# at-wat/mcl_3dl

Hardware: AMD Instinct MI355X
Metric: particle·point evals/sec; filter-update Hz @ 4096 particles × 16k-pt scan (higher is better)
Workload: dtype f32

## Files before the change

### mcl_3dl_amd/capi.py

```python
import ctypes as C
import os

import numpy as np

_HERE = os.path.dirname(os.path.abspath(__file__))
LIB_PATH = os.environ.get("MCL3DL_HIP_LIB") or os.path.join(_HERE, "libmcl3dl_hip.so")

KERNEL_LIKELIHOOD, KERNEL_BEAM, KERNEL_PF, KERNEL_UPDATE, KERNEL_STAGE = 0, 1, 2, 3, 4
BEAM_STATUS = {0: "SHORT", 1: "HIT", 2: "LONG", 3: "TOTAL_REFLECTION"}

_f, _d, _sz, _u32, _u64, _i, _p = C.c_float, C.c_double, C.c_size_t, C.c_uint32, C.c_uint64, C.c_int, C.c_void_p

SIGNATURES = {
    "mcl3dl_hip_abi_version": (_i, []),
    "mcl3dl_hip_create": (_i, [C.POINTER(_p), _i]),
    "mcl3dl_hip_destroy": (None, [_p]),
    "mcl3dl_hip_last_error": (C.c_char_p, [_p]),
    "mcl3dl_hip_set_stream": (_i, [_p, _p]),
    "mcl3dl_hip_get_stream": (_p, [_p]),
    "mcl3dl_hip_synchronize": (_i, [_p]),
    "mcl3dl_hip_set_map": (_i, [_p, _p, _p, _sz, _u64, _p]),
    "mcl3dl_hip_set_likelihood_params": (_i, [_p, _f, _f, _f]),
    "mcl3dl_hip_set_beam_params": (_i, [_p, _f, _f, _f, _f, _f, _f, _f, _u32, _f, _u32, _i]),
    "mcl3dl_hip_set_beam_raycast": (_i, [_p, _i]),
# ... 929 lines not shown
    def pf_partial_device(self, d_weight, d_lik, d_beam, d_extra, d_ratio, n_p, d_packed, rank=0, world=1):
        self._check(self.lib.mcl3dl_hip_pf_partial_device(self.h, _ptr(d_weight), _ptr(d_lik), _ptr(d_beam),
                                                          _ptr(d_extra), _ptr(d_ratio), n_p, int(rank), int(world),
                                                          _ptr(d_packed)))

    def pf_apply_device(self, d_weight, n_p, d_packed, d_stats4, world=1):
        self._check(self.lib.mcl3dl_hip_pf_apply_device(self.h, _ptr(d_weight), n_p, int(world), _ptr(d_packed),
                                                        _ptr(d_stats4)))

    def set_kernel_timing(self, enable):
        self._check(self.lib.mcl3dl_hip_set_kernel_timing(self.h, int(bool(enable))))

    def reset_kernel_time(self):
        self._check(self.lib.mcl3dl_hip_reset_kernel_time(self.h))

    def kernel_time(self, kernel_id):
        ms, n = C.c_double(0), C.c_uint64(0)
        self._check(self.lib.mcl3dl_hip_get_kernel_time(self.h, kernel_id, C.byref(ms), C.byref(n)))
        return float(ms.value), int(n.value)

    def workload_stats(self, d_pose, n_p):
        st = np.zeros(6, np.float64)
        self._check(self.lib.mcl3dl_hip_workload_stats(self.h, _ptr(d_pose), n_p, _ptr(st)))
        return dict(sum_k=st[0], evals=st[1], dda_steps=st[2], dda_occupied=st[3], dda_tested=st[4], rays=st[5])

    def memory_footprint(self):
        b = np.zeros(8, np.uint64)
        self._check(self.lib.mcl3dl_hip_memory_footprint(self.h, _ptr(b)))
        return dict(lik_points=int(b[0]), lik_cells=int(b[1]), dda_bits=int(b[2]), dda_voxels=int(b[3]),
                    dda_points=int(b[4]), cand_table=int(b[5]), cand_start=int(b[6]), cand_points=int(b[7]))

    def set_option(self, name, value):
        self._check(self.lib.mcl3dl_hip_set_option(self.h, name.encode(), float(value)))

    def get_option(self, name):
        v = C.c_double(0)
        self._check(self.lib.mcl3dl_hip_get_option(self.h, name.encode(), C.byref(v)))
        return float(v.value)

    def index_stats(self):
        s = np.zeros(8, np.float64)
        self._check(self.lib.mcl3dl_hip_index_stats(self.h, _ptr(s)))
        return dict(bricks=int(s[0]), preliminary=int(s[1]), candidates=int(s[2]), build_ms=float(s[3]),
                    voxels_with_candidates=int(s[4]), voxels_with_overflow=int(s[5]), overflow_records=int(s[6]),
                    voxel_ratio=float(s[7]), voxels_over8=int(self.get_option("cand_voxels_over8")),
                    record_parts=int(self.get_option("cand_record_parts_in_use")),
                    packed_words=int(self.get_option("cand_packed_active")),
                    deferred_overflow=int(self.get_option("lik_defer_active")))
```

### mcl_3dl_amd/csrc/host_context.h

```cpp
#pragma once

namespace
{
struct DevBuf
{
  void* p = nullptr;
  size_t cap = 0;
  bool view = false;
  DevBuf() = default;
  DevBuf(const DevBuf&) = delete;
  DevBuf& operator=(const DevBuf&) = delete;
  ~DevBuf()
  {
    if (p && !view)
      (void)hipFree(p);
  }
  template <typename T>
  T* as() const
  {
    return static_cast<T*>(p);
  }
};

struct OrderedScan
// ... 89 lines not shown
  struct PinnedBlock
  {
    char* p;
    size_t bytes;
  };
  std::vector<PinnedBlock> pinned;
  bool is_pinned(const void* q, size_t bytes) const
  {
    const char* c = static_cast<const char*>(q);
    for (const PinnedBlock& b : pinned)
      if (c >= b.p && c + bytes <= b.p + b.bytes)
        return true;
    return false;
  }
  bool cand_aniso_active = false;
  double index_budget_bytes = 0.0;
  double cand_need_bytes = 0.0;
  double cand_edge_ratio[3] = { 0.5, 0.5, 0.5 };
  uint32_t cand_parts = 4;
  int n_cus = 256;
  double cand_over8 = 0;
  DevBuf cand_table, cand_start, cand_pts, cand_rec, cand_ovf;
  DevBuf cand_all_pts;
  CompileParams cand_cp{};
  long long cand_n_table = 0;
  uint32_t cand_n_bricks = 0, cand_n_ovf = 0, cand_ovf_leaked = 0;
  uint64_t cand_ovf_compactions = 0;
  size_t cand_n_points = 0;
  RecGrid rg{};
  double cand_stats[8] = { 0, 0, 0, 0, 0, 0, 0, 0 };
  DevBuf dda_bits, dda_start, dda_pts, dda_index;
  DevBuf dda_ov_key, dda_ov_pts, dda_ov_idx;
  bool dda_overlay_ok = false;
  uint64_t dda_overlay_updates = 0;
  DdaGeom dda_geom{};
  DevBuf map_dev;
  bool map_dev_valid = false;
  size_t map_dev_n = 0;
  double grid_build_ms[2] = { 0, 0 };
  double grid_build_wall_ms[2] = { 0, 0 };
  DdaGrid dg{};
  uint64_t footprint[8] = { 0, 0, 0, 0, 0, 0, 0, 0 };

  DevBuf scan_lik, scan_beam, origins, pow_table;
  DevBuf beam_origin;
  size_t n_s = 0, n_b = 0, n_o = 0;
// ... 553 lines not shown
```

### mcl_3dl_amd/csrc/host_map_compilers.h

```cpp
#pragma once

namespace
{
int build_lik_grid(mcl3dl_hip_ctx* ctx);
int build_dda_grid(mcl3dl_hip_ctx* ctx);
int ensure_map_dev(mcl3dl_hip_ctx* ctx);
int cloud_minmax(mcl3dl_hip_ctx* ctx, const float4* pts, long long n, float* host6, unsigned long long* host_cnt);

void kd_ray_radii(const mcl3dl_hip_ctx* ctx, float* grid_min, float* r1, float* r2)
{
  const float mn = std::min({ ctx->map_grid[0], ctx->map_grid[1], ctx->map_grid[2] });
  const float mx = std::max({ ctx->map_grid[0], ctx->map_grid[1], ctx->map_grid[2] });
  *grid_min = mn;
  *r1 = static_cast<float>(std::sqrt(2.0) * mx / 2.0);
  *r2 = static_cast<float>(mn * 2 + std::sqrt(2.0) * mx / 2.0);
}

bool lik_cell_is_beams(const mcl3dl_hip_ctx* ctx)
{
  return !ctx->lik_params_set && ctx->beam_raycast == 1;
}

float lik_cell_edge(const mcl3dl_hip_ctx* ctx)
{
// ... 506 lines not shown
  if (want_packed >= 0)
    out->packed = want_packed;
  else
    out->packed = (can_bound && ctx->opt.cand_packed && ctx->opt.cand_bound) ? 2 : (can_pack && ctx->opt.cand_packed) ? 1 : 0;
  TRY(scratch_alloc(ctx, out->d_ovf_data, 64ull * (n_ovf ? n_ovf : 1)));
  {
    const long long words = 16ll * (n_ovf ? n_ovf : 1);
    uint32_t sentinel_bits;
    const float sentinel = REC_SENTINEL;
    memcpy(&sentinel_bits, &sentinel, sizeof(sentinel_bits));
    hipLaunchKernelGGL(mc_fill_u32, dim3(static_cast<unsigned>((words + 255) / 256)), dim3(256), 0, ctx->stream,
                       static_cast<uint32_t*>(out->d_ovf_data.p), sentinel_bits, words);
  }
  hipLaunchKernelGGL(mc_write_records, dim3(blocks_v), dim3(256), 0, ctx->stream, pts,
                     static_cast<const uint32_t*>(d_pstart.p), static_cast<const uint32_t*>(d_prelim.p),
                     static_cast<const uint32_t*>(d_count.p), static_cast<const uint32_t*>(d_ovf.p), rec_out,
                     static_cast<float*>(out->d_ovf_data.p), n_vox, cap, out->packed, cp, bxyz,
                     static_cast<double>(ctx->match_dist_min));
  HIP_TRY(hipGetLastError());
  out->n_ovf = n_ovf;
  return 0;
}

constexpr int RC_OVER_BUDGET = 1;

int build_cand_grid_at(mcl3dl_hip_ctx* ctx, double voxel_ratio, uint32_t cap = 4)
{
  const unsigned long long rec_bytes = 16ull * cap;
  const size_t n = ctx->map_xyz.size() / 3;
  EventPairRaii evs;
  HIP_TRY(hipEventCreate(&evs.a));
  HIP_TRY(hipEventCreate(&evs.b));
  const hipEvent_t ev0 = evs.a, ev1 = evs.b;
  HIP_TRY(hipEventRecord(ev0, ctx->stream));
  TRY(ensure_map_dev(ctx));
  TRY(ensure(ctx, ctx->cand_all_pts, sizeof(float4) * n));
  hipLaunchKernelGGL(grid_rescale_kernel, dim3(static_cast<unsigned>((n + 255) / 256)), dim3(256), 0, ctx->stream,
                     ctx->map_dev.as<float4>(), static_cast<long long>(n), ctx->weight[0], ctx->weight[1], ctx->weight[2],
                     ctx->has_weight ? 1 : 0, ctx->cand_all_pts.as<float4>());
  float mm[6];
  unsigned long long n_finite = 0;
  TRY(cloud_minmax(ctx, ctx->cand_all_pts.as<float4>(), static_cast<long long>(n), mm, &n_finite));
  if (n_finite != n)
    return ctx->fail(-3, "%llu map point(s) are not finite", static_cast<unsigned long long>(n) - n_finite);
  const float* mn = mm;
  const float* mx = mm + 3;
// ... 17 lines not shown
  uint32_t n_bricks = 0;
  TRY(d2h(ctx, &n_bricks, static_cast<uint32_t*>(d_scan.p) + n_table, sizeof(uint32_t)));
  TRY(sync_stream(ctx));
  if (n_bricks == 0 || n_bricks > (1u << 22))
    return ctx->fail(-4, "candidate index: %u bricks", n_bricks);
  ctx->cand_need_bytes = static_cast<double>(rec_bytes) * 512.0 * n_bricks;
  if (ctx->opt.lik_index == 2 && ctx->index_budget_bytes > 0.0 && ctx->cand_need_bytes > ctx->index_budget_bytes)
    return RC_OVER_BUDGET;
  TRY(ensure(ctx, ctx->cand_table, sizeof(int) * (n_table + 1)));
  int* table = ctx->cand_table.as<int>();
  hipLaunchKernelGGL(mc_brick_ids, dim3(static_cast<unsigned>((n_table + 255) / 256)), dim3(256), 0, ctx->stream,
                     static_cast<const int*>(d_flag.p), static_cast<const uint32_t*>(d_scan.p), table, n_table);
  HIP_TRY(hipMemsetAsync(table + n_table, 0xff, sizeof(int), ctx->stream));
  TRY(scratch_alloc(ctx, d_bxyz, sizeof(int) * 3 * n_bricks));
  hipLaunchKernelGGL(mc_brick_coords, dim3(static_cast<unsigned>((n_table + 255) / 256)), dim3(256), 0, ctx->stream,
                     table, cp.nbx, cp.nby, n_table, static_cast<int*>(d_bxyz.p));
  const long long n_vox = static_cast<long long>(n_bricks) * 512;
  const bool records = ctx->opt.lik_index == 2;
  if (records)
    TRY(ensure(ctx, ctx->cand_rec, rec_bytes * static_cast<size_t>(n_vox)));
  CompileOutput co;
  TRY(compile_bricks(ctx, cp, pts, table, static_cast<const int*>(d_bxyz.p), n_bricks, records,
                     records ? ctx->cand_rec.as<float>() : nullptr, &co, cap));
  const unsigned long long total = co.total, kept = co.kept;
  ctx->cand_cp = cp;
  ctx->cand_n_table = n_table;
  ctx->cand_n_bricks = n_bricks;
  ctx->cand_n_points = n;
  if (records)
  {
    const uint32_t n_ovf = co.n_ovf;
    TRY(ensure(ctx, ctx->cand_ovf, 64ull * (n_ovf ? n_ovf : 1)));
    HIP_TRY(hipMemcpyAsync(ctx->cand_ovf.p, co.d_ovf_data.p, 64ull * (n_ovf ? n_ovf : 1), hipMemcpyDeviceToDevice,
                           ctx->stream));
    ctx->cand_n_ovf = n_ovf;
    ctx->cand_ovf_leaked = 0;
    HIP_TRY(hipEventRecord(ev1, ctx->stream));
    TRY(sync_stream(ctx));
    float ms2 = 0.f;
    HIP_TRY(hipEventSynchronize(ev1));
    HIP_TRY(hipEventElapsedTime(&ms2, ev0, ev1));
    RecGrid& g = ctx->rg;
    g.brick_table = table;
    g.rec = ctx->cand_rec.as<float4>();
    g.ovf = ctx->cand_ovf.as<float4>();
    g.ox = cp.ox;
// ... 239 lines not shown
                       c2, static_cast<const float4*>(dst), static_cast<int*>(d_dirty.p));
  }
  const unsigned blocks_tab = static_cast<unsigned>((n_table + 1 + 255) / 256);
  TRY(scratch_alloc(ctx, d_newflag, sizeof(uint32_t) * (n_table + 1)));
  TRY(scratch_alloc(ctx, d_dirtyrank, sizeof(uint32_t) * (n_table + 1)));
  hipLaunchKernelGGL(mc_new_brick_flags, dim3(blocks_tab), dim3(256), 0, ctx->stream, static_cast<const int*>(d_dirty.p),
                     ctx->cand_table.as<int>(), static_cast<uint32_t*>(d_newflag.p), n_table);
  HIP_TRY(hipMemsetAsync(d_dirtyrank.p, 0, sizeof(uint32_t) * (n_table + 1), ctx->stream));
  HIP_TRY(hipMemcpyAsync(d_dirtyrank.p, d_dirty.p, sizeof(int) * n_table, hipMemcpyDeviceToDevice, ctx->stream));
  TRY(device_exclusive_scan(ctx, static_cast<uint32_t*>(d_newflag.p), n_table + 1));
  TRY(device_exclusive_scan(ctx, static_cast<uint32_t*>(d_dirtyrank.p), n_table + 1));
  uint32_t n_new = 0, n_dirty = 0;
  TRY(d2h(ctx, &n_new, static_cast<uint32_t*>(d_newflag.p) + n_table, sizeof(uint32_t)));
  TRY(d2h(ctx, &n_dirty, static_cast<uint32_t*>(d_dirtyrank.p) + n_table, sizeof(uint32_t)));
  TRY(sync_stream(ctx));
  const uint32_t n_bricks_old = ctx->cand_n_bricks;
  if (n_dirty == 0)
  {
    if (stats5)
      stats5[5] = 6;
    ctx->cand_n_points = n_total;
    return 0;
  }
  if (static_cast<unsigned long long>(n_bricks_old) + n_new > (1u << 22))
  {
    if (stats5)
      stats5[5] = 5;
    ctx->cand_dirty = true;
    return 0;
  }
  if (ctx->cand_ovf_leaked > std::max<uint32_t>(4096u, ctx->cand_n_ovf / 2))
    TRY(compact_overflow(ctx));
  const uint32_t n_bricks = n_bricks_old + n_new;
  const uint32_t cap = ctx->cand_parts;
  const unsigned long long rec_bytes = 16ull * cap;
  TRY(ensure_keep(ctx, ctx->cand_rec, rec_bytes * 512 * n_bricks_old, rec_bytes * 512 * n_bricks));
  TRY(scratch_alloc(ctx, d_sub_table, sizeof(int) * n_table));
  TRY(scratch_alloc(ctx, d_sub_main, sizeof(int) * n_dirty));
  TRY(scratch_alloc(ctx, d_sub_bxyz, sizeof(int) * 3 * n_dirty));
  hipLaunchKernelGGL(mc_dirty_tables, dim3(blocks_tab), dim3(256), 0, ctx->stream, static_cast<const int*>(d_dirty.p),
                     static_cast<const uint32_t*>(d_newflag.p), static_cast<const uint32_t*>(d_dirtyrank.p), n_bricks_old,
                     cp.nbx, cp.nby, n_table, ctx->cand_table.as<int>(), static_cast<int*>(d_sub_table.p),
                     static_cast<int*>(d_sub_main.p), static_cast<int*>(d_sub_bxyz.p));
  cp.n_points = static_cast<int>(n_total);
  TRY(scratch_alloc(ctx, d_relflag, sizeof(uint32_t) * (n_total + 1)));
  hipLaunchKernelGGL(mc_relevant_points, dim3(static_cast<unsigned>((n_total + 1 + 255) / 256)), dim3(256), 0, ctx->stream,
                     cp, ctx->cand_all_pts.as<float4>(), static_cast<const int*>(d_dirty.p),
                     static_cast<uint32_t*>(d_relflag.p));
  TRY(device_exclusive_scan(ctx, static_cast<uint32_t*>(d_relflag.p), static_cast<long long>(n_total) + 1));
  uint32_t n_rel = 0;
  TRY(d2h(ctx, &n_rel, static_cast<uint32_t*>(d_relflag.p) + n_total, sizeof(uint32_t)));
  TRY(sync_stream(ctx));
  TRY(scratch_alloc(ctx, d_rel, sizeof(float4) * (n_rel ? n_rel : 1)));
  hipLaunchKernelGGL(mc_compact_points, dim3(static_cast<unsigned>((n_total + 255) / 256)), dim3(256), 0, ctx->stream,
                     ctx->cand_all_pts.as<float4>(), static_cast<const uint32_t*>(d_relflag.p), static_cast<int>(n_total),
                     static_cast<float4*>(d_rel.p));
  const long long n_sub_vox = static_cast<long long>(n_dirty) * 512;
  TRY(scratch_alloc(ctx, d_subrec, rec_bytes * static_cast<size_t>(n_sub_vox)));
  cp.n_points = static_cast<int>(n_rel);
  CompileOutput co;
  {
    const int rc = compile_bricks(ctx, cp, static_cast<const float4*>(d_rel.p), static_cast<const int*>(d_sub_table.p),
                                  static_cast<const int*>(d_sub_bxyz.p), n_dirty, true, static_cast<float*>(d_subrec.p), &co,
                                  cap, word_format(ctx->rg), ctx->cand_n_ovf);
    if (rc == 1)
    {
// ... 2 lines not shown
      ctx->cand_dirty = true;
      return 0;
    }
    if (rc != 0)
      return rc;
  }
  const uint32_t ovf_base = ctx->cand_n_ovf;
  if (co.n_ovf)
  {
    TRY(ensure_keep(ctx, ctx->cand_ovf, 64ull * ovf_base, 64ull * (static_cast<size_t>(ovf_base) + co.n_ovf)));
    HIP_TRY(hipMemcpyAsync(ctx->cand_ovf.as<char>() + 64ull * ovf_base, co.d_ovf_data.p, 64ull * co.n_ovf,
                           hipMemcpyDeviceToDevice, ctx->stream));
  }
  TempBuf d_orphan;
  TRY(scratch_alloc(ctx, d_orphan, sizeof(unsigned long long)));
  HIP_TRY(hipMemsetAsync(d_orphan.p, 0, sizeof(unsigned long long), ctx->stream));
  hipLaunchKernelGGL(mc_install_records, dim3(static_cast<unsigned>((n_sub_vox + 255) / 256)), dim3(256), 0, ctx->stream,
                     static_cast<const float4*>(d_subrec.p), static_cast<const int*>(d_sub_main.p), ovf_base, n_bricks_old,
                     n_sub_vox, ctx->cand_rec.as<float4>(), static_cast<unsigned long long*>(d_orphan.p), cap, ctx->rg.packed,
                     ctx->rg.count_shift, ctx->rg.count_is_records);
  HIP_TRY(hipGetLastError());
  unsigned long long orphaned = 0;
  TRY(d2h(ctx, &orphaned, d_orphan.p, sizeof(orphaned)));
  HIP_TRY(hipEventRecord(ev1, ctx->stream));
  TRY(sync_stream(ctx));
  float ms = 0.f;
  HIP_TRY(hipEventSynchronize(ev1));
  HIP_TRY(hipEventElapsedTime(&ms, ev0, ev1));
  ctx->cand_n_bricks = n_bricks;
  ctx->cand_n_ovf = ovf_base + co.n_ovf;
  ctx->cand_ovf_leaked += static_cast<uint32_t>(orphaned);
  ctx->cand_n_points = n_total;
  ctx->rg.brick_table = ctx->cand_table.as<int>();
  ctx->rg.rec = ctx->cand_rec.as<float4>();
  ctx->rg.ovf = ctx->cand_ovf.as<float4>();
  ctx->rg.off32_ok = (rec_bytes * 512 * n_bricks < (1ull << 32)) ? 1 : 0;
  ctx->rg.rec_bytes32 = bytes32(rec_bytes * 512 * n_bricks);
  ctx->rg.ovf_bytes32 = bytes32(64ull * (ctx->cand_n_ovf ? ctx->cand_n_ovf : 1));
  ctx->footprint[6] = rec_bytes * 512 * n_bricks;
  ctx->footprint[7] = 64ull * ctx->cand_n_ovf;
  ctx->cand_stats[0] = n_bricks;
  ctx->cand_stats[6] = ctx->cand_n_ovf;
  if (stats5)
  {
    stats5[0] = n_dirty;
    stats5[1] = n_new;
// ... 9 lines not shown
```

### mcl_3dl_amd/csrc/host_measure.h

```cpp
#pragma once
#include <type_traits>

namespace
{
int ensure_structures(mcl3dl_hip_ctx* ctx, bool need_lik, bool need_dda, bool need_cells = false)
{
  if (!ctx->has_map)
    return ctx->fail(-5, "no map: call mcl3dl_hip_set_map first");
  bool built = false;
  if (need_lik && ctx->opt.lik_index == 0 && !need_cells && !ctx->lik_params_set && (ctx->lik_cell_from_beam || lik_cell_is_beams(ctx)))
  {
    ctx->lik_params_set = true;
    if (ctx->lik_cell_from_beam)
      ctx->lik_dirty = ctx->lik_base_dirty = true;
  }
  if (need_lik && (ctx->opt.lik_index == 0 || need_cells) && ctx->lik_dirty)
  {
    TRY(build_lik_grid(ctx));
    built = true;
  }
  if (need_lik && ctx->opt.lik_index >= 1 && !need_cells && ctx->cand_dirty)
  {
    TRY(build_cand_grid(ctx));
    built = true;
// ... 961 lines not shown
  const int np = static_cast<int>(n_p);
  if (ctx->n_s > 0)
    TRY(ensure(ctx, ctx->tested, sizeof(double) * n_p));
  if (ctx->n_b > 0)
  {
    long long n_rays = 0, blocks = 0;
    TRY(prepare_beam(ctx, n_p, &n_rays, &blocks));
    TRY(ensure(ctx, ctx->ray_stats, sizeof(RayStats)));
    const bool counters_clean = ctx->penalty_clean_n >= n_p;
    ctx->penalty_clean_n = 0;
    if (!counters_clean)
      zero_penalty(ctx, np, ctx->stream);
    HIP_TRY(hipMemsetAsync(ctx->ray_stats.p, 0, sizeof(RayStats), ctx->stream));
    hipLaunchKernelGGL((beam_kernel<true>), dim3(static_cast<unsigned>(blocks)), dim3(256), 0, ctx->stream, d_pose,
                       ctx->scan_beam.as<float4>(), static_cast<int>(ctx->n_b), ctx->origins.as<float4>(), n_rays, ctx->dg,
                       beam_params(ctx), ctx->penalty.as<unsigned>(), ctx->ray_stats.as<RayStats>(),
                       static_cast<const BeamOrigin*>(nullptr), static_cast<int>(ctx->n_o));
  }
  HIP_TRY(hipGetLastError());
  if (ctx->n_s > 0)
    hipLaunchKernelGGL((likelihood_kernel<256, 0, true>), dim3(np), dim3(256), 0, ctx->stream, d_pose, ctx->scan_lik.as<float4>(),
                       static_cast<int>(ctx->n_s), ctx->lg, ctx->rg, lik_params(ctx), nullptr, nullptr, ctx->tested.as<double>(), 0);
  HIP_TRY(hipGetLastError());
  std::vector<double> tested(ctx->n_s ? n_p : 0);
  RayStats rs{ 0, 0, 0 };
  if (ctx->n_s)
    TRY(d2h(ctx, tested.data(), ctx->tested.p, sizeof(double) * n_p));
  if (ctx->n_b)
    TRY(d2h(ctx, &rs, ctx->ray_stats.p, sizeof(RayStats)));
  TRY(sync_stream(ctx));
  stats6[0] = std::accumulate(tested.begin(), tested.end(), 0.0);
  stats6[1] = static_cast<double>(n_p) * static_cast<double>(ctx->n_s);
  stats6[2] = static_cast<double>(rs.steps);
  stats6[3] = static_cast<double>(rs.occupied);
  stats6[4] = static_cast<double>(rs.tested);
  stats6[5] = static_cast<double>(n_p) * static_cast<double>(ctx->n_b);
  return 0;
}

bool pf_float_order(const mcl3dl_hip_ctx* ctx, size_t n_p);

int launch_update_small(mcl3dl_hip_ctx* ctx, const float* d_pose, size_t n_p, float* d_weight, const float* d_extra,
                        float* d_lik, float* d_ratio, float* d_beam, float* d_stats4, const PfEmit* ho = nullptr)
{
  if (!ctx->opt.update_small || n_p == 0 || ctx->n_b > 256 || ctx->opt.strict_order == 3 || !ctx->has_scan || !d_lik || !d_ratio || !d_beam)
    return 0;
  if (n_p > static_cast<size_t>(ctx->opt.update_small_max))
    return 0;
  if (ctx->beam_raycast == 1 && ctx->n_b > 0)
    return 0;
  const int np = static_cast<int>(n_p), ns = static_cast<int>(ctx->n_s);
  const LikMode mode = ns > 0 ? lik_mode(ctx, np, ns) : LikMode{};
  if (ns > 0 && (mode.tiled || lik_small_applies(ctx, mode, np, ns)))
// ... 66 lines not shown
```

### mcl_3dl_amd/csrc/likelihood_kernels.h

```cpp
#pragma once
#include <hip/hip_runtime.h>
#include <stdint.h>

#include "device_math.h"
#include "float_chain.h"
#include "map_structs.h"
#pragma clang fp contract(off)

namespace mcl3dl
{
template <bool STATS>
__device__ inline float nearest_d2(const LikGrid& g, float qx, float qy, float qz, unsigned& n_tested)
{
  const float fx = floorf((qx - g.ox) * g.inv_cell);
  const float fy = floorf((qy - g.oy) * g.inv_cell);
  const float fz = floorf((qz - g.oz) * g.inv_cell);
  float best = 3.0e38f;
  if (!(fx >= 1.0f && fy >= 1.0f && fz >= 1.0f && fx <= static_cast<float>(g.nx - 2) &&
        fy <= static_cast<float>(g.ny - 2) && fz <= static_cast<float>(g.nz - 2)))
    return best;
  const int cx = static_cast<int>(fx), cy = static_cast<int>(fy), cz = static_cast<int>(fz);
  uint32_t rs[9], re[9];
#pragma unroll
  for (int r = 0; r < 9; ++r)
// ... 98 lines not shown
         __umul24(static_cast<uint32_t>(vy >> 3), static_cast<uint32_t>(g.nbx)) + static_cast<uint32_t>(vx >> 3);
  else
    ti = (static_cast<uint32_t>(vz >> 3) * static_cast<uint32_t>(g.nby) + static_cast<uint32_t>(vy >> 3)) *
             static_cast<uint32_t>(g.nbx) + static_cast<uint32_t>(vx >> 3);
  sub = ((((static_cast<uint32_t>(vz) & 7u) << 3) | (static_cast<uint32_t>(vy) & 7u)) << 3) | (static_cast<uint32_t>(vx) & 7u);
  return static_cast<unsigned>(vx) < static_cast<unsigned>(g.nvx) && static_cast<unsigned>(vy) < static_cast<unsigned>(g.nvy) &&
         static_cast<unsigned>(vz) < static_cast<unsigned>(g.nvz);
}

__device__ inline float rec_overflow_min(const RecGrid& g, float qx, float qy, float qz, uint32_t n_records, uint32_t ext,
                                         float best)
{
  const float4* o = g.ovf + 4 * static_cast<size_t>(ext);
  for (uint32_t j = 0; j < 4u * n_records; ++j)
  {
    const float4 c = o[j];
    const float d = d2_simple(qx, qy, qz, c.x, c.y, c.z);
    best = d < best ? d : best;
  }
  return best;
}

template <bool STATS>
__device__ inline float nearest_d2_rec(const RecGrid& g, float qx, float qy, float qz, unsigned& n_tested)
{
  float best = 3.0e38f;
  uint32_t ti, sub;
  if (!rec_locate(g, qx, qy, qz, ti, sub))
    return best;
  const int b = g.brick_table[ti];
  if (b < 0)
    return best;
  const uint32_t cap = static_cast<uint32_t>(g.rec_parts);
  const float4* r = g.rec + static_cast<size_t>(cap) * ((static_cast<uint32_t>(b) << 9) | sub);
  const float4 r0 = r[0], r1 = r[1];
  const uint32_t w0 = __float_as_uint(r0.w);
  const uint32_t field = g.packed ? w0 >> g.count_shift : w0;
  const uint32_t n_records = rec_overflow_records(field, cap, g.count_is_records);
  if (!g.count_is_records && field == 0)
    return best;
  if (STATS)
    n_tested += g.count_is_records ? cap + 4u * n_records : field;
  best = fminf(d2_simple(qx, qy, qz, r0.x, r0.y, r0.z), d2_simple(qx, qy, qz, r1.x, r1.y, r1.z));
  for (uint32_t k = 2; k < cap; ++k)
  {
    const float4 c = r[k];
    best = fminf(best, d2_simple(qx, qy, qz, c.x, c.y, c.z));
  }
  if (n_records && !(g.bound_step > 0.0f && best <= rec_bound2(g, w0)))
    best = rec_overflow_min(g, qx, qy, qz, n_records, g.packed ? (w0 & rec_ext_mask(g)) : __float_as_uint(r1.w), best);
  return best;
}


__device__ inline Vec3f qrot_trim(const Quat q, const Vec3f v)
{
  const float px = (q.w * v.x + q.y * v.z) - q.z * v.y;
  const float py = (q.w * v.y + q.z * v.x) - q.x * v.z;
// ... 191 lines not shown
      best = (more && m < best) ? m : best;
    }
  }
  return best;
}

__device__ inline float sqrt_in_radius(float x)
{
  float s = __builtin_amdgcn_sqrtf(x);
  const float s_dn = __uint_as_float(__float_as_uint(s) - 1u), s_up = __uint_as_float(__float_as_uint(s) + 1u);
  const float vp = __builtin_fmaf(-s_dn, s, x), vs = __builtin_fmaf(-s_up, s, x);
  s = (vp <= 0.0f) ? s_dn : s;
  s = (vs > 0.0f) ? s_up : s;
  return s;
}

__device__ inline float eval_coop(const RecGrid& rg, const LikParams& prm, const Vec3f pos, const Quat rot, const float4 v,
                                  bool have_point, int lane, bool& matched)
{
  const Vec3f tp = vadd(qrot_trim(rot, Vec3f{ v.x, v.y, v.z }), pos);
  const float qx = tp.x * prm.wx, qy = tp.y * prm.wy, qz = tp.z * prm.wz;
  uint32_t ti, sub;
  const bool inside = rec_locate(rg, qx, qy, qz, ti, sub) && have_point;
  const int b = rg.brick_table[inside ? ti : rg.ti_empty];
  const bool valid = b >= 0;
  float dist = -1.0f;
  if (wave_any(valid))
  {
    const uint32_t rec = (static_cast<uint32_t>(b) << 9) | sub;
    const uint32_t vrec = rg.rec_bytes32 ? rec : (valid ? rec : 0u);
    const float d2 = rec_min_d2_quad(rg, qx, qy, qz, vrec, valid, lane);
    if (valid && d2 < prm.r2)
    {
      const float s = sqrt_in_radius(d2);
      dist = lik_dist(prm, s);
    }
  }
  matched = !(dist < 0.0f);
  return lik_term(prm, dist, matched);
}

template <int BLOCK, int MODE, bool STATS>
__device__ __forceinline__ void lik_particle(const Vec3f pos, const Quat rot, const float4* __restrict__ scan, int n_s,
                                             const LikGrid& g, const RecGrid& rg, const LikParams& prm,
                                             int coop, double& sum_out, unsigned& num_out, unsigned& tested_out,
                                             const uint32_t* __restrict__ perm = nullptr, float* s_row = nullptr)
{
  double acc = 0.0;
  unsigned num = 0;
  unsigned tested = 0;
  const bool rows = !STATS && s_row != nullptr;
  if (rows)
// ... 108 lines not shown
  {
    if (out_lik)
      out_lik[p] = static_cast<float>(a);
    if (out_ratio)
      out_ratio[p] = static_cast<float>(n) / static_cast<float>(n_s);
    if (STATS && out_tested)
      out_tested[p] = static_cast<double>(tt);
  }
}

template <int BLOCK, int MODE, bool STATS>
__global__ __launch_bounds__(BLOCK) void likelihood_kernel(const float* __restrict__ pose7,
                                                           const float4* __restrict__ scan, int n_s, LikGrid g,
                                                           RecGrid rg, LikParams prm,
                                                           float* __restrict__ out_lik,
                                                           float* __restrict__ out_ratio,
                                                           double* __restrict__ out_tested, int coop,
                                                           const uint32_t* __restrict__ perm = nullptr)
{
  likelihood_particle_body<BLOCK, MODE, STATS>(static_cast<int>(blockIdx.x), pose7, scan, n_s, g, rg, prm, out_lik, out_ratio,
                                               out_tested, coop, perm);
}

template <int W, int MODE>
__global__ __launch_bounds__(256) void likelihood_small_kernel(const float* __restrict__ pose7, int n_p,
                                                               const float4* __restrict__ scan, int n_s, LikGrid g,
                                                               RecGrid rg, LikParams prm,
                                                               float* __restrict__ out_lik, float* __restrict__ out_ratio,
                                                               int coop, const uint32_t* __restrict__ perm = nullptr)
{
  const long long gt = static_cast<long long>(blockIdx.x) * 256 + threadIdx.x;
  const long long p = gt / W;
  const int i = static_cast<int>(gt % W);
  float term = 0.0f;
  unsigned num = 0;
  if (MODE == 2 && coop)
  {
    const bool have = p < n_p && i < n_s;
    const float* ps = pose7 + 7 * (p < n_p ? p : 0);
    const Vec3f pos = { ps[0], ps[1], ps[2] };
    const Quat rot = qnormalized(Quat{ ps[3], ps[4], ps[5], ps[6] });
    const float4 v = scan[i < n_s ? i : 0];
    bool matched;
    term = eval_coop(rg, prm, pos, rot, v, have, static_cast<int>(threadIdx.x & 63), matched);
    num = matched ? 1u : 0u;
  }
// ... 71 lines not shown

__device__ inline unsigned long long chain_pack(uint32_t value, uint32_t tag)
{
  return (static_cast<unsigned long long>(tag) << 32) | value;
}

constexpr int CHAIN_POLL_MAX = 1 << 20;
constexpr int DEFER_QCAP = 96;

struct DeferQueue
{
  uint32_t word[4][DEFER_QCAP];
  uint16_t who[4][DEFER_QCAP];
};

__device__ inline float eval_coop_first(const RecGrid& rg, const LikParams& prm, const Vec3f pos, const Quat rot, const float4 v,
                                        bool have_point, int lane, bool& matched, bool& over, float& best, uint32_t& mine,
                                        unsigned long long& over_m)
{
  const Vec3f tp = vadd(qrot_trim(rot, Vec3f{ v.x, v.y, v.z }), pos);
  const float qx = tp.x * prm.wx, qy = tp.y * prm.wy, qz = tp.z * prm.wz;
  uint32_t ti, sub;
  const bool inside = rec_locate(rg, qx, qy, qz, ti, sub) && have_point;
  const int b = rg.brick_table[inside ? ti : rg.ti_empty];
  const bool valid = b >= 0;
  float dist = -1.0f;
  over = false;
  over_m = 0ull;
  best = 0.0f;
  mine = 0u;
  const unsigned long long valid_m = __builtin_amdgcn_ballot_w64(valid);
  if (valid_m != 0ull)
  {
    const uint32_t rec = (static_cast<uint32_t>(b) << 9) | sub;
    const uint32_t vrec = rg.rec_bytes32 ? rec : (valid ? rec : 0u);
    uint32_t w[4];
    best = quad_round(rg.rec, rg.rec_bytes32, vrec, qx, qy, qz, lane & 3, w);
    mine = own_word(w, lane & 3);
    over_m = valid_m & lanes_gt_u32(mine, rg.over_thr);
    if (rg.bound_step > 0.0f && over_m != 0ull)
    {
      asm volatile("");
      over_m &= __builtin_amdgcn_fcmpf(best, rec_bound2(rg, mine), 2 );
    }
    over = __builtin_amdgcn_inverse_ballot_w64(over_m);
    if (valid && !over && best < prm.r2)
    {
      const float s = sqrt_in_radius(best);
      dist = lik_dist(prm, s);
    }
  }
  matched = !(dist < 0.0f);
  return lik_term(prm, dist, matched);
}

template <int G, int LD>
__device__ inline void defer_drain(const RecGrid& rg, const LikParams& prm, const float (&s_pose)[G][8], float (&s_term)[G][LD],
// ... 507 lines not shown
```

### mcl_3dl_amd/csrc/map_compiler.h

```cpp
#pragma once
#include <hip/hip_runtime.h>
#include <stdint.h>

namespace mcl3dl
{
struct CompileParams
{
  float ox, oy, oz, inv_ex, inv_ey, inv_ez;
  double ex, ey, ez;
  double grow;
  double r2_hi;
  double margin;
  int rx, ry, rz;
  int nvx, nvy, nvz, nbx, nby, nbz;
  int n_points;
};

__device__ inline int3 voxel_of(const CompileParams& c, const float4 p)
{
  return make_int3(static_cast<int>(floorf((p.x - c.ox) * c.inv_ex)), static_cast<int>(floorf((p.y - c.oy) * c.inv_ey)),
                   static_cast<int>(floorf((p.z - c.oz) * c.inv_ez)));
}

__device__ inline long long brick_index(const CompileParams& c, int vx, int vy, int vz)
{
// ... 489 lines not shown


constexpr float REC_SENTINEL = 1.0e18f;
constexpr uint32_t REC_EXT_BITS = 26u, REC_EXT_MASK = (1u << REC_EXT_BITS) - 1u, REC_COUNT_MAX = 63u;
constexpr uint32_t REC2_EXT_BITS = 22u, REC2_COUNT_SHIFT = 28u, REC2_BOUND_MAX = 63u;

struct RecGrid
{
  const int32_t* brick_table;
  const float4* rec;
  const float4* ovf;
  float ox, oy, oz, inv_ex, inv_ey, inv_ez;
  int nvx, nvy, nvz, nbx, nby, nbz;
  int mul24_ok;
  int off32_ok;
  uint32_t rec_bytes32, ovf_bytes32;
  int rec_parts;
  uint32_t ti_empty;
  int packed;
  uint32_t count_shift, ext_bits;
  int count_is_records;
  uint32_t over_thr;
  float bound_step;
};

__host__ __device__ inline uint32_t rec_ext_mask(const RecGrid& g)
{
  return (1u << g.ext_bits) - 1u;
}
__host__ __device__ inline uint32_t rec_overflow_records(uint32_t field, uint32_t cap, int count_is_records)
{
  return count_is_records ? field : (field > cap ? (field - cap + 3u) / 4u : 0u);
}
__device__ inline float rec_bound2(const RecGrid& g, uint32_t w)
{
  const float bd = static_cast<float>((w >> REC2_EXT_BITS) & REC2_BOUND_MAX) * g.bound_step;
  return bd * bd;
}

__global__ __launch_bounds__(256) void mc_count_overflow(const uint32_t* __restrict__ kept_count, uint32_t* __restrict__ n_ovf,
                                                         long long n_vox, unsigned long long* __restrict__ hist3, uint32_t cap)
{
  __shared__ unsigned long long s_h[5];
  if (threadIdx.x < 5)
    s_h[threadIdx.x] = 0ull;
  __syncthreads();
// ... 88 lines not shown
    {
      const float4 p = pts[prelim[src + k] & 0x7fffffffu];
      const uint32_t j = k - cap;
      float* slot = o + 4 * j;
      slot[0] = p.x;
      slot[1] = p.y;
      slot[2] = p.z;
    }
  }
}

__global__ void mc_new_brick_flags(const int* __restrict__ dirty, const int* __restrict__ table, uint32_t* __restrict__ new_flag,
                                   long long n_table)
{
  const long long i = static_cast<long long>(blockIdx.x) * blockDim.x + threadIdx.x;
  if (i > n_table)
    return;
  new_flag[i] = (i < n_table && dirty[i] && table[i] < 0) ? 1u : 0u;
}

__global__ void mc_dirty_tables(const int* __restrict__ dirty, const uint32_t* __restrict__ new_rank,
                                const uint32_t* __restrict__ dirty_rank, uint32_t n_bricks_old, int nbx, int nby,
                                long long n_table, int* __restrict__ table, int* __restrict__ sub_table,
                                int* __restrict__ sub_main, int* __restrict__ sub_bxyz)
{
  const long long i = static_cast<long long>(blockIdx.x) * blockDim.x + threadIdx.x;
  if (i >= n_table)
    return;
  if (!dirty[i])
  {
    sub_table[i] = -1;
    return;
  }
  int id = table[i];
  if (id < 0)
  {
    id = static_cast<int>(n_bricks_old + new_rank[i]);
    table[i] = id;
  }
  const int sub = static_cast<int>(dirty_rank[i]);
  sub_table[i] = sub;
  sub_main[sub] = id;
  const long long plane = static_cast<long long>(nbx) * nby;
  sub_bxyz[3 * sub + 0] = static_cast<int>(i % nbx);
  sub_bxyz[3 * sub + 1] = static_cast<int>((i / nbx) % nby);
  sub_bxyz[3 * sub + 2] = static_cast<int>(i / plane);
}

__global__ void mc_relevant_points(CompileParams c, const float4* __restrict__ pts, const int* __restrict__ dirty,
                                   uint32_t* __restrict__ flag)
{
  const int pi = blockIdx.x * blockDim.x + threadIdx.x;
  if (pi > c.n_points)
    return;
  if (pi == c.n_points)
  {
    flag[pi] = 0;
    return;
  }
  const int3 v = voxel_of(c, pts[pi]);
  const int x0 = max(v.x - c.rx, 0) >> 3, x1 = min(v.x + c.rx, c.nvx - 1) >> 3;
  const int y0 = max(v.y - c.ry, 0) >> 3, y1 = min(v.y + c.ry, c.nvy - 1) >> 3;
  const int z0 = max(v.z - c.rz, 0) >> 3, z1 = min(v.z + c.rz, c.nvz - 1) >> 3;
  uint32_t f = 0;
  for (int z = z0; z <= z1; ++z)
    for (int y = y0; y <= y1; ++y)
      for (int x = x0; x <= x1; ++x)
        f |= dirty[(static_cast<long long>(z) * c.nby + y) * c.nbx + x] ? 1u : 0u;
  flag[pi] = f;
// ... 168 lines not shown
```

Measured before the change: 298.2 billion.

## Encode per-brick empty-slab masks in brick table to skip record loads

Packs an axis-aligned 8-slab emptiness mask and axis selector into the upper bits of each brick table entry, computed at map compile time from per-voxel kept counts. Likelihood kernels test the mask and treat queries that fall into a proven-empty slab as misses, so they skip loading the voxel's candidate records. Brick ids are limited to 21 bits when masks are on, which forces a rebuild path for large maps. It also adds a stats tally kernel and diagnostics.

```diff
diff --git a/mcl_3dl_amd/capi.py b/mcl_3dl_amd/capi.py
--- a/mcl_3dl_amd/capi.py
+++ b/mcl_3dl_amd/capi.py
@@ -975,7 +975,9 @@
     def workload_stats(self, d_pose, n_p):
         st = np.zeros(6, np.float64)
         self._check(self.lib.mcl3dl_hip_workload_stats(self.h, _ptr(d_pose), n_p, _ptr(st)))
-        return dict(sum_k=st[0], evals=st[1], dda_steps=st[2], dda_occupied=st[3], dda_tested=st[4], rays=st[5])
+        return dict(sum_k=st[0], evals=st[1], dda_steps=st[2], dda_occupied=st[3], dda_tested=st[4], rays=st[5],
+                    slab_proven_empty=self.get_option("slab_evals_proven_empty"),
+                    slab_occupied=self.get_option("slab_evals_occupied"))
 
     def memory_footprint(self):
         b = np.zeros(8, np.uint64)
@@ -999,4 +1001,7 @@
                     voxel_ratio=float(s[7]), voxels_over8=int(self.get_option("cand_voxels_over8")),
                     record_parts=int(self.get_option("cand_record_parts_in_use")),
                     packed_words=int(self.get_option("cand_packed_active")),
-                    deferred_overflow=int(self.get_option("lik_defer_active")))
+                    deferred_overflow=int(self.get_option("lik_defer_active")),
+                    slab_masks=int(self.get_option("slab_masks_active")),
+                    empty_slabs=int(self.get_option("slab_empty_slabs")),
+                    empty_voxels=int(self.get_option("slab_empty_voxels")))
diff --git a/mcl_3dl_amd/csrc/brick_entry.h b/mcl_3dl_amd/csrc/brick_entry.h
--- /dev/null
+++ b/mcl_3dl_amd/csrc/brick_entry.h
@@ -0,0 +1,74 @@
+#pragma once
+#include <stdint.h>
+
+#if defined(__HIPCC__) || defined(__CUDACC__)
+#define BRICK_ENTRY_FN __host__ __device__ inline
+#else
+#define BRICK_ENTRY_FN inline
+#endif
+
+namespace mcl3dl
+{
+constexpr uint32_t BRICK_ID_BITS = 21u;
+constexpr uint32_t BRICK_ID_MASK = (1u << BRICK_ID_BITS) - 1u;
+constexpr uint32_t BRICK_ID_MASK_PLAIN = 0x7fffffffu;
+constexpr uint32_t BRICK_MASKED_MAX = 1u << BRICK_ID_BITS;
+constexpr uint32_t BRICK_SLAB_SHIFT = BRICK_ID_BITS;
+constexpr uint32_t BRICK_AXIS_SHIFT = BRICK_ID_BITS + 8u;
+
+BRICK_ENTRY_FN int32_t brick_entry_encode(uint32_t id, uint32_t axis, uint32_t empty)
+{
+  return static_cast<int32_t>((id & BRICK_ID_MASK) | ((empty & 0xffu) << BRICK_SLAB_SHIFT) | ((axis & 3u) << BRICK_AXIS_SHIFT));
+}
+BRICK_ENTRY_FN uint32_t brick_entry_id(int32_t e, uint32_t id_mask)
+{
+  return static_cast<uint32_t>(e) & id_mask;
+}
+BRICK_ENTRY_FN uint32_t brick_entry_axis(int32_t e)
+{
+  return (static_cast<uint32_t>(e) >> BRICK_AXIS_SHIFT) & 3u;
+}
+BRICK_ENTRY_FN uint32_t brick_entry_empty_mask(int32_t e)
+{
+  return (static_cast<uint32_t>(e) >> BRICK_SLAB_SHIFT) & 0xffu;
+}
+BRICK_ENTRY_FN uint32_t brick_layer(uint32_t sub, uint32_t axis)
+{
+  return (sub >> (axis + (axis << 1))) & 7u;
+}
+BRICK_ENTRY_FN bool brick_entry_proven_empty(int32_t e, uint32_t sub, uint32_t slab_on)
+{
+  const uint32_t u = static_cast<uint32_t>(e);
+  const uint32_t layer = brick_layer(sub, (u >> BRICK_AXIS_SHIFT) & 3u);
+  return ((u >> layer) & (slab_on << BRICK_SLAB_SHIFT)) != 0u;
+}
+
+BRICK_ENTRY_FN void slab_occupy(uint32_t sub, uint32_t (&occ)[3])
+{
+  occ[0] |= 1u << (sub & 7u);
+  occ[1] |= 1u << ((sub >> 3) & 7u);
+  occ[2] |= 1u << ((sub >> 6) & 7u);
+}
+BRICK_ENTRY_FN uint32_t slab_popcount8(uint32_t m)
+{
+  m = (m & 0x55u) + ((m >> 1) & 0x55u);
+  m = (m & 0x33u) + ((m >> 2) & 0x33u);
+  return (m & 0x0fu) + (m >> 4);
+}
+BRICK_ENTRY_FN uint32_t slab_pick(const uint32_t (&occ)[3])
+{
+  uint32_t axis = 0;
+  for (uint32_t a = 1; a < 3; ++a)
+    if (slab_popcount8(occ[a] & 0xffu) < slab_popcount8(occ[axis] & 0xffu))
+      axis = a;
+  return (axis << 8) | (~occ[axis] & 0xffu);
+}
+BRICK_ENTRY_FN uint32_t slab_pick_from_counts(const uint32_t* count512)
+{
+  uint32_t occ[3] = { 0u, 0u, 0u };
+  for (uint32_t sub = 0; sub < 512u; ++sub)
+    if (count512[sub] != 0u)
+      slab_occupy(sub, occ);
+  return slab_pick(occ);
+}
+}
diff --git a/mcl_3dl_amd/csrc/host_context.h b/mcl_3dl_amd/csrc/host_context.h
--- a/mcl_3dl_amd/csrc/host_context.h
+++ b/mcl_3dl_amd/csrc/host_context.h
@@ -135,6 +135,9 @@
   double cand_over8 = 0;
   DevBuf cand_table, cand_start, cand_pts, cand_rec, cand_ovf;
   DevBuf cand_all_pts;
+  DevBuf cand_brick_info;
+  double slab_empty_voxels = 0, slab_empty_slabs = 0;
+  double slab_evals_proven_empty = -1, slab_evals_occupied = -1;
   CompileParams cand_cp{};
   long long cand_n_table = 0;
   uint32_t cand_n_bricks = 0, cand_n_ovf = 0, cand_ovf_leaked = 0;
diff --git a/mcl_3dl_amd/csrc/host_map_compilers.h b/mcl_3dl_amd/csrc/host_map_compilers.h
--- a/mcl_3dl_amd/csrc/host_map_compilers.h
+++ b/mcl_3dl_amd/csrc/host_map_compilers.h
@@ -552,6 +552,26 @@
   return 0;
 }
 
+int write_slab_masks(mcl3dl_hip_ctx* ctx, const CompileParams& cp, const CompileOutput& co, const int* bxyz, const int* main_id,
+                     uint32_t n_bricks, uint32_t n_total)
+{
+  hipLaunchKernelGGL(mc_slab_masks, dim3(n_bricks), dim3(64), 0, ctx->stream, static_cast<const uint32_t*>(co.d_count.p), bxyz,
+                     main_id, cp.nbx, cp.nby, n_bricks, ctx->cand_table.as<int32_t>(), ctx->cand_brick_info.as<uint32_t>(),
+                     static_cast<int>(ctx->rg.slab_on));
+  TempBuf d_totals;
+  TRY(scratch_alloc(ctx, d_totals, 2 * sizeof(unsigned long long)));
+  HIP_TRY(hipMemsetAsync(d_totals.p, 0, 2 * sizeof(unsigned long long), ctx->stream));
+  hipLaunchKernelGGL(mc_slab_totals, dim3(std::min(64u, (n_total + 255u) / 256u)), dim3(256), 0, ctx->stream,
+                     ctx->cand_brick_info.as<uint32_t>(), n_total, static_cast<unsigned long long*>(d_totals.p));
+  HIP_TRY(hipGetLastError());
+  unsigned long long totals[2] = { 0, 0 };
+  TRY(d2h(ctx, totals, d_totals.p, sizeof(totals)));
+  TRY(sync_stream(ctx));
+  ctx->slab_empty_voxels = static_cast<double>(totals[0]);
+  ctx->slab_empty_slabs = static_cast<double>(totals[1]);
+  return 0;
+}
+
 constexpr int RC_OVER_BUDGET = 1;
 
 int build_cand_grid_at(mcl3dl_hip_ctx* ctx, double voxel_ratio, uint32_t cap = 4)
@@ -615,6 +635,13 @@
   CompileOutput co;
   TRY(compile_bricks(ctx, cp, pts, table, static_cast<const int*>(d_bxyz.p), n_bricks, records,
                      records ? ctx->cand_rec.as<float>() : nullptr, &co, cap));
+  ctx->rg.slab_on = n_bricks < BRICK_MASKED_MAX ? 1u : 0u;
+  ctx->rg.id_mask = ctx->rg.slab_on ? BRICK_ID_MASK : BRICK_ID_MASK_PLAIN;
+  if (records)
+  {
+    TRY(ensure(ctx, ctx->cand_brick_info, sizeof(uint32_t) * n_bricks));
+    TRY(write_slab_masks(ctx, cp, co, static_cast<const int*>(d_bxyz.p), nullptr, n_bricks, n_bricks));
+  }
   const unsigned long long total = co.total, kept = co.kept;
   ctx->cand_cp = cp;
   ctx->cand_n_table = n_table;
@@ -900,7 +927,8 @@
     ctx->cand_n_points = n_total;
     return 0;
   }
-  if (static_cast<unsigned long long>(n_bricks_old) + n_new > (1u << 22))
+  if (static_cast<unsigned long long>(n_bricks_old) + n_new > (1u << 22) ||
+      (ctx->rg.slab_on && static_cast<unsigned long long>(n_bricks_old) + n_new >= BRICK_MASKED_MAX))
   {
     if (stats5)
       stats5[5] = 5;
@@ -919,7 +947,7 @@
   hipLaunchKernelGGL(mc_dirty_tables, dim3(blocks_tab), dim3(256), 0, ctx->stream, static_cast<const int*>(d_dirty.p),
                      static_cast<const uint32_t*>(d_newflag.p), static_cast<const uint32_t*>(d_dirtyrank.p), n_bricks_old,
                      cp.nbx, cp.nby, n_table, ctx->cand_table.as<int>(), static_cast<int*>(d_sub_table.p),
-                     static_cast<int*>(d_sub_main.p), static_cast<int*>(d_sub_bxyz.p));
+                     static_cast<int*>(d_sub_main.p), static_cast<int*>(d_sub_bxyz.p), ctx->rg.id_mask);
   cp.n_points = static_cast<int>(n_total);
   TRY(scratch_alloc(ctx, d_relflag, sizeof(uint32_t) * (n_total + 1)));
   hipLaunchKernelGGL(mc_relevant_points, dim3(static_cast<unsigned>((n_total + 1 + 255) / 256)), dim3(256), 0, ctx->stream,
@@ -968,6 +996,9 @@
   HIP_TRY(hipGetLastError());
   unsigned long long orphaned = 0;
   TRY(d2h(ctx, &orphaned, d_orphan.p, sizeof(orphaned)));
+  TRY(ensure_keep(ctx, ctx->cand_brick_info, sizeof(uint32_t) * n_bricks_old, sizeof(uint32_t) * n_bricks));
+  TRY(write_slab_masks(ctx, cp, co, static_cast<const int*>(d_sub_bxyz.p), static_cast<const int*>(d_sub_main.p), n_dirty,
+                       n_bricks));
   HIP_TRY(hipEventRecord(ev1, ctx->stream));
   TRY(sync_stream(ctx));
   float ms = 0.f;
diff --git a/mcl_3dl_amd/csrc/host_measure.h b/mcl_3dl_amd/csrc/host_measure.h
--- a/mcl_3dl_amd/csrc/host_measure.h
+++ b/mcl_3dl_amd/csrc/host_measure.h
@@ -1007,6 +1007,19 @@
     hipLaunchKernelGGL((likelihood_kernel<256, 0, true>), dim3(np), dim3(256), 0, ctx->stream, d_pose, ctx->scan_lik.as<float4>(),
                        static_cast<int>(ctx->n_s), ctx->lg, ctx->rg, lik_params(ctx), nullptr, nullptr, ctx->tested.as<double>(), 0);
   HIP_TRY(hipGetLastError());
+  TempBuf d_slab;
+  const bool slab_tally = ctx->n_s > 0 && ctx->opt.lik_index == 2 && !ctx->cand_dirty;
+  if (slab_tally)
+  {
+    TRY(scratch_alloc(ctx, d_slab, 2 * sizeof(unsigned long long)));
+    HIP_TRY(hipMemsetAsync(d_slab.p, 0, 2 * sizeof(unsigned long long), ctx->stream));
+    hipLaunchKernelGGL((slab_tally_kernel<256>), dim3(np), dim3(256), 0, ctx->stream, d_pose, ctx->scan_lik.as<float4>(),
+                       static_cast<int>(ctx->n_s), ctx->rg, lik_params(ctx), static_cast<unsigned long long*>(d_slab.p));
+    HIP_TRY(hipGetLastError());
+  }
+  unsigned long long slab2[2] = { 0, 0 };
+  if (slab_tally)
+    TRY(d2h(ctx, slab2, d_slab.p, sizeof(slab2)));
   std::vector<double> tested(ctx->n_s ? n_p : 0);
   RayStats rs{ 0, 0, 0 };
   if (ctx->n_s)
@@ -1014,6 +1027,8 @@
   if (ctx->n_b)
     TRY(d2h(ctx, &rs, ctx->ray_stats.p, sizeof(RayStats)));
   TRY(sync_stream(ctx));
+  ctx->slab_evals_proven_empty = slab_tally ? static_cast<double>(slab2[0]) : -1.0;
+  ctx->slab_evals_occupied = slab_tally ? static_cast<double>(slab2[1]) : -1.0;
   stats6[0] = std::accumulate(tested.begin(), tested.end(), 0.0);
   stats6[1] = static_cast<double>(n_p) * static_cast<double>(ctx->n_s);
   stats6[2] = static_cast<double>(rs.steps);
diff --git a/mcl_3dl_amd/csrc/likelihood_kernels.h b/mcl_3dl_amd/csrc/likelihood_kernels.h
--- a/mcl_3dl_amd/csrc/likelihood_kernels.h
+++ b/mcl_3dl_amd/csrc/likelihood_kernels.h
@@ -144,18 +144,27 @@
 }
 
 template <bool STATS>
-__device__ inline float nearest_d2_rec(const RecGrid& g, float qx, float qy, float qz, unsigned& n_tested)
+__device__ inline float nearest_d2_rec(const RecGrid& g, float qx, float qy, float qz, unsigned& n_tested,
+                                       unsigned* n_slab = nullptr)
 {
   float best = 3.0e38f;
   uint32_t ti, sub;
   if (!rec_locate(g, qx, qy, qz, ti, sub))
     return best;
-  const int b = g.brick_table[ti];
-  if (b < 0)
+  const int e = g.brick_table[ti];
+  if (e < 0)
+    return best;
+  const bool proven_empty = brick_entry_proven_empty(e, sub, g.slab_on);
+  if (!STATS && proven_empty)
     return best;
   const uint32_t cap = static_cast<uint32_t>(g.rec_parts);
-  const float4* r = g.rec + static_cast<size_t>(cap) * ((static_cast<uint32_t>(b) << 9) | sub);
+  const float4* r = g.rec + static_cast<size_t>(cap) * ((brick_entry_id(e, g.id_mask) << 9) | sub);
   const float4 r0 = r[0], r1 = r[1];
+  if (STATS && n_slab)
+  {
+    n_slab[0] += proven_empty ? 1u : 0u;
+    n_slab[1] += r0.x != REC_SENTINEL ? 1u : 0u;
+  }
   const uint32_t w0 = __float_as_uint(r0.w);
   const uint32_t field = g.packed ? w0 >> g.count_shift : w0;
   const uint32_t n_records = rec_overflow_records(field, cap, g.count_is_records);
@@ -393,12 +402,13 @@
   const float qx = tp.x * prm.wx, qy = tp.y * prm.wy, qz = tp.z * prm.wz;
   uint32_t ti, sub;
   const bool inside = rec_locate(rg, qx, qy, qz, ti, sub) && have_point;
-  const int b = rg.brick_table[inside ? ti : rg.ti_empty];
+  const int e = rg.brick_table[inside ? ti : rg.ti_empty];
+  const int b = brick_entry_proven_empty(e, sub, rg.slab_on) ? -1 : e;
   const bool valid = b >= 0;
   float dist = -1.0f;
   if (wave_any(valid))
   {
-    const uint32_t rec = (static_cast<uint32_t>(b) << 9) | sub;
+    const uint32_t rec = (brick_entry_id(b, rg.id_mask) << 9) | sub;
     const uint32_t vrec = rg.rec_bytes32 ? rec : (valid ? rec : 0u);
     const float d2 = rec_min_d2_quad(rg, qx, qy, qz, vrec, valid, lane);
     if (valid && d2 < prm.r2)
@@ -553,6 +563,38 @@
                                                out_tested, coop, perm);
 }
 
+template <int BLOCK>
+__global__ __launch_bounds__(BLOCK) void slab_tally_kernel(const float* __restrict__ pose7, const float4* __restrict__ scan,
+                                                           int n_s, RecGrid rg, LikParams prm,
+                                                           unsigned long long* __restrict__ out2)
+{
+  const float* ps = pose7 + 7 * static_cast<size_t>(blockIdx.x);
+  const Vec3f pos = { ps[0], ps[1], ps[2] };
+  const Quat rot = qnormalized(Quat{ ps[3], ps[4], ps[5], ps[6] });
+  unsigned tally[2] = { 0u, 0u }, tested = 0u;
+  for (int i = threadIdx.x; i < n_s; i += BLOCK)
+  {
+    const float4 v = scan[i];
+    const Vec3f t = vadd(qrot(rot, Vec3f{ v.x, v.y, v.z }), pos);
+    float qx = t.x, qy = t.y, qz = t.z;
+    if (prm.has_weight)
+    {
+      qx = t.x * prm.wx;
+      qy = t.y * prm.wy;
+      qz = t.z * prm.wz;
+    }
+    (void)nearest_d2_rec<true>(rg, qx, qy, qz, tested, tally);
+  }
+  const unsigned a = wave_sum(tally[0]), b = wave_sum(tally[1]);
+  if ((threadIdx.x & 63) == 0)
+  {
+    if (a)
+      atomicAdd(&out2[0], static_cast<unsigned long long>(a));
+    if (b)
+      atomicAdd(&out2[1], static_cast<unsigned long long>(b));
+  }
+}
+
 template <int W, int MODE>
 __global__ __launch_bounds__(256) void likelihood_small_kernel(const float* __restrict__ pose7, int n_p,
                                                                const float4* __restrict__ scan, int n_s, LikGrid g,
@@ -670,7 +712,8 @@
   const float qx = tp.x * prm.wx, qy = tp.y * prm.wy, qz = tp.z * prm.wz;
   uint32_t ti, sub;
   const bool inside = rec_locate(rg, qx, qy, qz, ti, sub) && have_point;
-  const int b = rg.brick_table[inside ? ti : rg.ti_empty];
+  const int e = rg.brick_table[inside ? ti : rg.ti_empty];
+  const int b = brick_entry_proven_empty(e, sub, rg.slab_on) ? -1 : e;
   const bool valid = b >= 0;
   float dist = -1.0f;
   over = false;
@@ -680,7 +723,7 @@
   const unsigned long long valid_m = __builtin_amdgcn_ballot_w64(valid);
   if (valid_m != 0ull)
   {
-    const uint32_t rec = (static_cast<uint32_t>(b) << 9) | sub;
+    const uint32_t rec = (brick_entry_id(b, rg.id_mask) << 9) | sub;
     const uint32_t vrec = rg.rec_bytes32 ? rec : (valid ? rec : 0u);
     uint32_t w[4];
     best = quad_round(rg.rec, rg.rec_bytes32, vrec, qx, qy, qz, lane & 3, w);
diff --git a/mcl_3dl_amd/csrc/map_compiler.h b/mcl_3dl_amd/csrc/map_compiler.h
--- a/mcl_3dl_amd/csrc/map_compiler.h
+++ b/mcl_3dl_amd/csrc/map_compiler.h
@@ -1,6 +1,8 @@
 #pragma once
 #include <hip/hip_runtime.h>
 #include <stdint.h>
+
+#include "brick_entry.h"
 
 namespace mcl3dl
 {
@@ -536,6 +538,7 @@
   int count_is_records;
   uint32_t over_thr;
   float bound_step;
+  uint32_t id_mask, slab_on;
 };
 
 __host__ __device__ inline uint32_t rec_ext_mask(const RecGrid& g)
@@ -670,7 +673,7 @@
 __global__ void mc_dirty_tables(const int* __restrict__ dirty, const uint32_t* __restrict__ new_rank,
                                 const uint32_t* __restrict__ dirty_rank, uint32_t n_bricks_old, int nbx, int nby,
                                 long long n_table, int* __restrict__ table, int* __restrict__ sub_table,
-                                int* __restrict__ sub_main, int* __restrict__ sub_bxyz)
+                                int* __restrict__ sub_main, int* __restrict__ sub_bxyz, uint32_t id_mask)
 {
   const long long i = static_cast<long long>(blockIdx.x) * blockDim.x + threadIdx.x;
   if (i >= n_table)
@@ -681,11 +684,8 @@
     return;
   }
   int id = table[i];
-  if (id < 0)
-  {
-    id = static_cast<int>(n_bricks_old + new_rank[i]);
-    table[i] = id;
-  }
+  id = id < 0 ? static_cast<int>(n_bricks_old + new_rank[i]) : static_cast<int>(brick_entry_id(id, id_mask));
+  table[i] = id;
   const int sub = static_cast<int>(dirty_rank[i]);
   sub_table[i] = sub;
   sub_main[sub] = id;
@@ -693,6 +693,56 @@
   sub_bxyz[3 * sub + 0] = static_cast<int>(i % nbx);
   sub_bxyz[3 * sub + 1] = static_cast<int>((i / nbx) % nby);
   sub_bxyz[3 * sub + 2] = static_cast<int>(i / plane);
+}
+
+__global__ __launch_bounds__(64) void mc_slab_masks(const uint32_t* __restrict__ kept_count, const int* __restrict__ bxyz,
+                                                    const int* __restrict__ main_id, int nbx, int nby, uint32_t n_bricks,
+                                                    int32_t* __restrict__ table, uint32_t* __restrict__ brick_info, int masks_on)
+{
+  const uint32_t s = blockIdx.x, t = threadIdx.x;
+  if (s >= n_bricks)
+    return;
+  uint32_t occ[3] = { 0u, 0u, 0u };
+  uint32_t filled = 0;
+  for (uint32_t k = 0; k < 8u; ++k)
+  {
+    const uint32_t sub = k * 64u + t;
+    if (kept_count[static_cast<size_t>(s) * 512u + sub] != 0u)
+    {
+      slab_occupy(sub, occ);
+      ++filled;
+    }
+  }
+  for (int m = 32; m > 0; m >>= 1)
+  {
+    occ[0] |= static_cast<uint32_t>(__shfl_xor(static_cast<int>(occ[0]), m));
+    occ[1] |= static_cast<uint32_t>(__shfl_xor(static_cast<int>(occ[1]), m));
+    occ[2] |= static_cast<uint32_t>(__shfl_xor(static_cast<int>(occ[2]), m));
+    filled += static_cast<uint32_t>(__shfl_xor(static_cast<int>(filled), m));
+  }
+  if (t != 0)
+    return;
+  const uint32_t id = main_id ? static_cast<uint32_t>(main_id[s]) : s;
+  const long long ti = (static_cast<long long>(bxyz[3 * s + 2]) * nby + bxyz[3 * s + 1]) * nbx + bxyz[3 * s + 0];
+  const uint32_t pick = slab_pick(occ);
+  const uint32_t empty = masks_on ? (pick & 0xffu) : 0u;
+  table[ti] = masks_on ? brick_entry_encode(id, pick >> 8, empty) : static_cast<int32_t>(id);
+  brick_info[id] = (512u - filled) | (slab_popcount8(empty) << 16);
+}
+
+__global__ __launch_bounds__(256) void mc_slab_totals(const uint32_t* __restrict__ brick_info, uint32_t n_bricks,
+                                                      unsigned long long* __restrict__ totals)
+{
+  unsigned long long vox = 0, slabs = 0;
+  for (uint32_t i = blockIdx.x * blockDim.x + threadIdx.x; i < n_bricks; i += gridDim.x * blockDim.x)
+  {
+    vox += brick_info[i] & 0xffffu;
+    slabs += brick_info[i] >> 16;
+  }
+  if (vox)
+    atomicAdd(&totals[0], vox);
+  if (slabs)
+    atomicAdd(&totals[1], slabs);
 }
 
 __global__ void mc_relevant_points(CompileParams c, const float4* __restrict__ pts, const int* __restrict__ dirty,
```

Result: no change. 296.4 billion (-0.6%).
